# ZhiHuangHn/vtkCloudPoint

Measured on AMD Instinct MI355X. Metric: Mpoints/s DBSCAN+label @10M pts, higher is better.
Workload: dtype f64; 1 GPU; C4: 10000000-pt cloud (half uniform background, 200 Gaussian blobs), one monolithic DBImproved.dbscan, metric L1_2D, eps 0.1, minPts 10; mode=single, points_total=10000000, points_per_gpu=10000000, clusters=27380, resident_in_hbm=True

## Files before the change

### vtkcloudpoint_amd/csrc/gridbuild.hip

```cpp
#include <algorithm>
#include <mutex>
#include <unordered_map>

#include "grid_common.hpp"

using namespace vcpg;

namespace {

constexpr int PT = 1024;
constexpr int PCH_MIN = 8192;
constexpr int FT = 1024;
constexpr uint32_t MAXB = 8192;
constexpr uint32_t wcap(int) { return 4096u; }
constexpr uint32_t QUEUE_FROM = 32;

typedef float4 Rec;

template <int GD>
__device__ __forceinline__ Rec rec_make(const float* qf, uint32_t idx, uint32_t cell) {
  return GD == 2 ? make_float4(qf[0], qf[1], __uint_as_float(idx), __uint_as_float(cell))
                 : make_float4(qf[0], qf[1], qf[2], __uint_as_float(idx));
}
template <int GD>
// ... 27 lines not shown
  uint32_t nchunk;
};

inline int env_int(const char* name, int dflt, int lo, int hi) {
  const char* e = getenv(name);
  int v = e ? atoi(e) : dflt;
  return v < lo ? lo : v > hi ? hi : v;
}

inline PartGeom part_geom(int64_t n, uint32_t ncells) {
  static const int csh_max = env_int("VCP_CPB_LOG2", 14, 10, 14);
  static const int target = env_int("VCP_PART_CHUNKS", 256, 64, 8192);
  PartGeom p;
  int csh = csh_max;
  while (csh > 10 && ((uint64_t)ncells >> csh) * 4096ull < (uint64_t)n) csh--;
  p.csh = (uint32_t)csh;
  p.B = (uint32_t)((((uint64_t)ncells + 1) + ((1ull << p.csh) - 1)) >> p.csh);
  p.a = 0;
  while (((p.B + (1u << p.a) - 1u) >> p.a) > MAXB) p.a++;
  p.NS = (p.B + (1u << p.a) - 1u) >> p.a;
  int64_t chunk = (n + target - 1) / target;
  if (chunk < PCH_MIN) chunk = PCH_MIN;
  chunk = (chunk + PT - 1) / PT * PT;
  p.chunk = (uint32_t)chunk;
  p.nchunk = (uint32_t)((n + chunk - 1) / chunk);
  return p;
}

template <int GD, bool GROUPED>
__global__ __launch_bounds__(PT) void k_part_hist(const double* __restrict__ c, int64_t n, int stride, GridP g,
                                                 const int32_t* __restrict__ group, int glo, int ghi, uint32_t csh,
                                                 uint32_t B, uint32_t chunk, uint32_t nchunk,
                                                 uint32_t* __restrict__ counts, uint32_t* __restrict__ qcount,
                                                 uint32_t* __restrict__ ctcount) {
  extern __shared__ uint32_t h[];
  if (blockIdx.x == 0 && threadIdx.x == 0) {
    *qcount = 0u;
    ctcount[0] = 0u;
  }
  for (uint32_t k = threadIdx.x; k < B; k += PT) h[k] = 0;
  __syncthreads();
  const int64_t first = (int64_t)blockIdx.x * chunk;
  const int64_t last = min(first + (int64_t)chunk, n);
#pragma unroll 4
  for (int64_t i = first + threadIdx.x; i < last; i += PT) {
    if (GROUPED) {
      const int gg = group[i];
      if (gg < glo || gg >= ghi) continue;
    }
    float qf[3];
    atomicAdd(&h[point_cell<GD>(c, i, stride, g, qf) >> csh], 1u);
  }
  __syncthreads();
  for (uint32_t k = threadIdx.x; k < B; k += PT) counts[(size_t)k * nchunk + blockIdx.x] = h[k];
}

template <int GD, bool GROUPED>
__global__ __launch_bounds__(PT) void k_part_scatter(const double* __restrict__ c, int64_t n, int stride, GridP g,
                                                    const int32_t* __restrict__ group, int glo, int ghi, uint32_t csh,
                                                    uint32_t B, uint32_t chunk, uint32_t nchunk,
                                                    const uint32_t* __restrict__ base, Rec* __restrict__ rec,
                                                    uint32_t* __restrict__ pos) {
  extern __shared__ uint32_t h[];
  for (uint32_t k = threadIdx.x; k < B; k += PT) h[k] = base[(size_t)k * nchunk + blockIdx.x];
  __syncthreads();
  const int64_t first = (int64_t)blockIdx.x * chunk;
  const int64_t last = min(first + (int64_t)chunk, n);
#pragma unroll 4
  for (int64_t i = first + threadIdx.x; i < last; i += PT) {
    if (GROUPED) {
      const int gg = group[i];
      if (gg < glo || gg >= ghi) {
        if (pos) pos[i] = NONE;
        continue;
      }
    }
    float qf[3];
    const uint32_t cell = point_cell<GD>(c, i, stride, g, qf);
    rec[atomicAdd(&h[cell >> csh], 1u)] = rec_make<GD>(qf, (uint32_t)i, cell);
  }
}

__device__ __forceinline__ uint32_t padded(uint32_t i) { return i + (i >> 5); }

template <int GD, bool GROUPED, int NT = FT>
__device__ __forceinline__ void fine_flush(uint32_t s0, uint32_t m, const float* s32, const uint32_t* sidx,
                                           const uint32_t* __restrict__ ord, const uint8_t* __restrict__ in_classed,
                                           const int32_t* __restrict__ group, float* __restrict__ sorted32,
                                           uint32_t* __restrict__ sord, uint32_t* __restrict__ sidx_out,
                                           int32_t* __restrict__ sgroup, uint8_t* __restrict__ flags,
                                           uint32_t* __restrict__ pos) {
  if (GD == 2) {
    const float2* src = reinterpret_cast<const float2*>(s32);
    float2* dst = reinterpret_cast<float2*>(sorted32) + s0;
    for (uint32_t k = threadIdx.x; k < m; k += NT) dst[k] = src[k];
  } else {
    const float4* src = reinterpret_cast<const float4*>(s32);
    float4* dst = reinterpret_cast<float4*>(sorted32) + s0;
    for (uint32_t k = threadIdx.x; k < m; k += NT) dst[k] = src[k];
  }
  for (uint32_t k = threadIdx.x; k < m; k += NT) {
    const uint32_t i = sidx[k], p = s0 + k;
    sord[p] = ord ? ord[i] : i;
    if (sidx_out) sidx_out[p] = i;
    if (GROUPED) sgroup[p] = group[i];
    if (in_classed) flags[p] = in_classed[i] ? F_CLASSED : 0;
    if (pos) pos[i] = p;
  }
}

template <int GD>
__device__ __forceinline__ void stage_put(float* s32, uint32_t* sidx, uint32_t p, const Rec& r, uint32_t idx) {
  if (GD == 2) reinterpret_cast<float2*>(s32)[p] = make_float2(r.x, r.y);
  else reinterpret_cast<float4*>(s32)[p] = make_float4(r.x, r.y, r.z, 0.0f);
  sidx[p] = idx;
}

__device__ __forceinline__ void bucket_range(const uint32_t* __restrict__ bstart, uint32_t bstride, const uint32_t* __restrict__ total,
                                             uint32_t b, uint32_t B, uint32_t& s, uint32_t& e) {
  s = bstart[(size_t)b * bstride];
  e = (b + 1 < B) ? bstart[(size_t)(b + 1) * bstride] : *total;
}

template <int GD>
__global__ __launch_bounds__(FT) void k_part_split(const Rec* __restrict__ rec, Rec* __restrict__ rec2,
                                                  const uint32_t* __restrict__ base, const uint32_t* __restrict__ total,
                                                  uint32_t nchunk, uint32_t NS, uint32_t a, uint32_t csh, uint32_t B, GridP g,
                                                  uint32_t* __restrict__ bstart) {
  __shared__ uint32_t h[32];
  const uint32_t S = blockIdx.x;
  uint32_t s, e;
  bucket_range(base, nchunk, total, S, NS, s, e);
  const uint32_t subm = (1u << a) - 1u;
  if (threadIdx.x < 32) h[threadIdx.x] = 0u;
// ... 4 lines not shown
  }
  __syncthreads();
  if (threadIdx.x < 32) {
    const uint32_t v = h[threadIdx.x];
    uint32_t inc = v;
#pragma unroll
    for (int d = 1; d < 32; d <<= 1) {
      const uint32_t t = __shfl_up(inc, d, 64);
      if ((int)threadIdx.x >= d) inc += t;
    }
    const uint32_t first = s + inc - v;
    h[threadIdx.x] = first;
    const uint32_t bk = (S << a) + threadIdx.x;
    if (threadIdx.x <= subm && bk <= B) bstart[bk] = first;
  }
  __syncthreads();
  for (uint32_t j = s + threadIdx.x; j < e; j += FT) {
    const Rec r = rec[j];
    uint32_t i;
    rec2[atomicAdd(&h[(rec_cell<GD>(r, g, i) >> csh) & subm], 1u)] = r;
  }
}

constexpr int FS = 512;
constexpr uint32_t scap(int gd) { return gd == 2 ? 2048u : 1536u; }
constexpr uint32_t SPOP = 128;

template <int GD, bool GROUPED>
__global__ __launch_bounds__(FS) void k_part_fine_small(const Rec* __restrict__ rec, const uint32_t* __restrict__ bstart,
                                                       uint32_t bstride, const uint32_t* __restrict__ total, uint32_t B,
                                                       uint32_t csh, GridP g, const uint32_t* __restrict__ ord,
                                                       const uint8_t* __restrict__ in_classed, const int32_t* __restrict__ group,
                                                       uint4* __restrict__ ctwords, uint32_t* __restrict__ ctdense,
                                                       uint32_t* __restrict__ ctcount, uint8_t* __restrict__ bstate,
                                                       float* __restrict__ sorted32, uint32_t* __restrict__ sord,
                                                       uint32_t* __restrict__ sidx_out, int32_t* __restrict__ sgroup,
                                                       uint8_t* __restrict__ flags, uint32_t* __restrict__ pos) {
  constexpr uint32_t FPR = GD == 2 ? 2 : 4;
  constexpr uint32_t SCAP = scap(GD);
  constexpr int SRPT = SCAP / FS;
  __shared__ uint32_t ws[512 + 2];
  __shared__ uint32_t wlo[512], whi[512];
  __shared__ uint16_t wpi[512];
  __shared__ uint8_t sci[SCAP];
  __shared__ __attribute__((aligned(16))) uint16_t st32[SPOP][32];
  __shared__ __attribute__((aligned(16))) float s32[SCAP * FPR];
  __shared__ uint32_t sidx[SCAP];
  __shared__ uint32_t wsum[FS / 64];
  __shared__ uint32_t s_np, s_dbase;
  const uint32_t b = blockIdx.x;
  uint32_t s, e;
  bucket_range(bstart, bstride, total, b, B, s, e);
  const uint32_t m = e - s;
  if (b + 1 == B && threadIdx.x == 0) ctcount[1] = *total;
  if (m > SCAP) {
    if (threadIdx.x == 0) bstate[b] = 1;
    return;
  }
  const uint32_t CPB = 1u << csh, NW = CPB >> 5, c0 = b << csh;
  const int lane = threadIdx.x & 63, w = threadIdx.x >> 6;
  for (uint32_t k = threadIdx.x; k < NW + 1; k += FS) ws[k] = 0u;
  __syncthreads();
  Rec r[SRPT];
  uint32_t idx[SRPT], lw[SRPT], ci[SRPT], rnk[SRPT];
#pragma unroll
  for (int k = 0; k < SRPT; k++) {
    const uint32_t j = s + (uint32_t)k * FS + threadIdx.x;
    lw[k] = NONE;
    if (j < e) {
      r[k] = rec[j];
      const uint32_t c = rec_cell<GD>(r[k], g, idx[k]) - c0;
      lw[k] = c >> 5;
      ci[k] = c & 31u;
      rnk[k] = atomicAdd(&ws[lw[k]], 1u);
    }
  }
  __syncthreads();
  {
    const uint32_t v = threadIdx.x < NW ? ws[threadIdx.x] : 0u;
    uint32_t inc = v;
#pragma unroll
    for (int d = 1; d < 64; d <<= 1) {
      const uint32_t t = __shfl_up(inc, d, 64);
      if (lane >= d) inc += t;
    }
    if (lane == 63) wsum[w] = inc;
    __syncthreads();
    uint32_t pre = inc - v;
    for (int k = 0; k < w; k++) pre += wsum[k];
// ... 6 lines not shown
    if (lw[k] != NONE) sci[ws[lw[k]] - s + rnk[k]] = (uint8_t)ci[k];
  __syncthreads();
  bool popl = false;
  uint32_t lo = 0u, hi = 0u;
  if (threadIdx.x < NW) {
    const uint32_t a = ws[threadIdx.x] - s, k = ws[threadIdx.x + 1] - s - a;
    if (k > 64u) {
      popl = true;
    } else {
      for (uint32_t i = 0; i < k; i++) {
        const uint32_t bit = 1u << sci[a + i];
        if (lo & hi & bit) continue;
        if (lo & bit) hi ^= bit;
        lo ^= bit;
      }
      popl = (lo & hi) != 0u;
    }
  }
  {
    const unsigned long long dm = __ballot(popl);
    if (lane == 0) wsum[w] = (uint32_t)__popcll(dm);
    __syncthreads();
    uint32_t before = (uint32_t)__popcll(dm & ((1ull << lane) - 1ull)), tot = 0;
    for (int k = 0; k < FS / 64; k++) {
      if (k < w) before += wsum[k];
      tot += wsum[k];
    }
    if (threadIdx.x == 0) s_np = tot;
    if (threadIdx.x < NW) wpi[threadIdx.x] = popl ? (uint16_t)before : (uint16_t)0xFFFFu;
  }
  __syncthreads();
  const uint32_t np = s_np;
  if (np > SPOP) {
    if (threadIdx.x == 0) bstate[b] = 1;
    return;
  }
  if (threadIdx.x == 0) {
    bstate[b] = 0;
    s_dbase = np ? atomicAdd(&ctcount[0], np) : 0u;
  }
  for (uint32_t k = threadIdx.x; k < np * 16u; k += FS) reinterpret_cast<uint32_t*>(&st32[0][0])[k] = 0u;
  if (threadIdx.x < NW && !popl) {
    wlo[threadIdx.x] = lo;
    whi[threadIdx.x] = hi;
  }
  __syncthreads();
#pragma unroll
  for (int k = 0; k < SRPT; k++)
    if (lw[k] != NONE && wpi[lw[k]] != 0xFFFFu) {
      uint16_t* c = &st32[wpi[lw[k]]][ci[k]];
      atomicAdd(reinterpret_cast<uint32_t*>(reinterpret_cast<uintptr_t>(c) & ~(uintptr_t)3), ((uintptr_t)c & 2) ? 0x10000u : 1u);
    }
  __syncthreads();
  {
    const uint32_t hw = threadIdx.x >> 5, li = threadIdx.x & 31u;
    for (uint32_t wd = hw; wd < NW; wd += FS / 32) {
      const uint32_t pi = wpi[wd];
      if (pi == 0xFFFFu) continue;
      const uint32_t c = st32[pi][li];
      uint32_t inc = c;
#pragma unroll
      for (int d = 1; d < 32; d <<= 1) {
        const uint32_t t = __shfl_up(inc, d, 32);
        if ((int)li >= d) inc += t;
      }
      const uint32_t first = ws[wd] + inc - c;
      st32[pi][li] = (uint16_t)(first - s);
      ctdense[(size_t)(s_dbase + pi) * 32u + li] = first;
      const uint32_t cs = min(c, 3u);
      const unsigned long long blo = __ballot(cs & 1u), bhi = __ballot(cs >> 1);
      const int sh = (threadIdx.x & 32) ? 32 : 0;
      if (li == 0) {
        wlo[wd] = (uint32_t)(blo >> sh);
        whi[wd] = (uint32_t)(bhi >> sh);
      }
    }
  }
  __syncthreads();
#pragma unroll
  for (int k = 0; k < SRPT; k++) {
    if (lw[k] == NONE) continue;
    const uint32_t pi = wpi[lw[k]];
    uint32_t p;
    if (pi != 0xFFFFu) {
      uint16_t* c = &st32[pi][ci[k]];
      const bool up = ((uintptr_t)c & 2) != 0;
      const uint32_t old = atomicAdd(reinterpret_cast<uint32_t*>(reinterpret_cast<uintptr_t>(c) & ~(uintptr_t)3), up ? 0x10000u : 1u);
      p = up ? old >> 16 : old & 0xFFFFu;
    } else {
      const uint32_t l = wlo[lw[k]], h = whi[lw[k]], below = (1u << ci[k]) - 1u;
      const uint32_t a = ws[lw[k]] - s;
      p = a + (uint32_t)__popc(l & below) + 2u * (uint32_t)__popc(h & below);
      if ((h >> ci[k]) & 1u)
        for (uint32_t i = 0; i < rnk[k]; i++) p += sci[a + i] == (uint8_t)ci[k] ? 1u : 0u;
    }
    stage_put<GD>(s32, sidx, p, r[k], idx[k]);
  }
  if (threadIdx.x < NW) {
    const size_t W = (size_t)(c0 >> 5) + threadIdx.x;
    const uint32_t pi = wpi[threadIdx.x];
    if (W < vcp_ct_words(g.ncells))
      ctwords[W] = make_uint4(wlo[threadIdx.x], whi[threadIdx.x], ws[threadIdx.x], pi != 0xFFFFu ? s_dbase + pi : NONE);
  }
  __syncthreads();
  fine_flush<GD, GROUPED, FS>(s, m, s32, sidx, ord, in_classed, group, sorted32, sord, sidx_out, sgroup, flags, pos);
}

template <int GD, bool GROUPED>
__global__ __launch_bounds__(FT) void k_part_fine(const Rec* __restrict__ rec, uint32_t* __restrict__ rk,
                                                 const uint32_t* __restrict__ bstart, uint32_t bstride,
                                                 const uint32_t* __restrict__ total, uint32_t B, uint32_t csh, GridP g,
                                                 const uint32_t* __restrict__ ord, const uint8_t* __restrict__ in_classed,
                                                 const int32_t* __restrict__ group, uint4* __restrict__ ctwords,
                                                 uint32_t* __restrict__ ctdense, uint32_t* __restrict__ ctcount,
                                                 float* __restrict__ sorted32, uint32_t* __restrict__ sord,
                                                 uint32_t* __restrict__ sidx_out, int32_t* __restrict__ sgroup,
                                                 uint8_t* __restrict__ flags, uint32_t* __restrict__ pos,
                                                 uint2* __restrict__ queue, uint32_t* __restrict__ qcount,
                                                 const uint8_t* __restrict__ bstate) {
  extern __shared__ __attribute__((aligned(16))) unsigned char lds[];
  __shared__ uint32_t wsum[FT / 64];
  __shared__ uint32_t w_lo[512], w_hi[512], w_slot[512];
  __shared__ uint32_t s_dbase;
  const uint32_t b = blockIdx.x;
  if (bstate[b] == 0) return;
  constexpr uint32_t WCAP = wcap(GD);
  constexpr uint32_t FPR = GD == 2 ? 2 : 4;
  const uint32_t CPB = 1u << csh;
  uint32_t* cnt = reinterpret_cast<uint32_t*>(lds);
  float* s32 = reinterpret_cast<float*>(lds + (((size_t)padded(CPB) + 4) & ~3ull) * 4);
  uint32_t* sidx = reinterpret_cast<uint32_t*>(s32 + (size_t)WCAP * FPR);
  const uint32_t c0 = b << csh;
  uint32_t s, e;
  bucket_range(bstart, bstride, total, b, B, s, e);
  const uint32_t m = e - s;
  const bool big = m > WCAP;
  for (uint32_t k = threadIdx.x; k < padded(CPB); k += FT) cnt[k] = 0;
  __syncthreads();
  for (uint32_t j = s + threadIdx.x; j < e; j += FT) {
    uint32_t i;
    uint32_t* slot = &cnt[padded(rec_cell<GD>(rec[j], g, i) - c0)];
    if (big) rk[j] = atomicAdd(slot, 1u);
    else atomicAdd(slot, 1u);
  }
  __syncthreads();
  const uint32_t PER = CPB / FT;
  const uint32_t first = threadIdx.x * PER;
  uint32_t loc = 0;
  for (uint32_t k = 0; k < PER; k++) loc += cnt[padded(first + k)];
  const int lane = threadIdx.x & 63, w = threadIdx.x >> 6;
  uint32_t inc = loc;
#pragma unroll
  for (int d = 1; d < 64; d <<= 1) {
    const uint32_t t = __shfl_up(inc, d, 64);
    if (lane >= d) inc += t;
  }
  if (lane == 63) wsum[w] = inc;
  __syncthreads();
  uint32_t pre = s + inc - loc;
  for (int k = 0; k < w; k++) pre += wsum[k];
  const uint32_t NW = CPB >> 5;
  uint32_t plo = 0u, phi = 0u;
  const uint32_t wstart = pre;
  {
    const uint32_t bit0 = first & 31u;
    for (uint32_t k = 0; k < PER; k++) {
      const uint32_t v = cnt[padded(first + k)];
      cnt[padded(first + k)] = pre;
      pre += v;
      const uint32_t c = min(v, 3u);
      plo |= (c & 1u) << (bit0 + k);
      phi |= (c >> 1) << (bit0 + k);
    }
    for (uint32_t d = 1; d < 32u / PER; d <<= 1) {
      plo |= (uint32_t)__shfl_xor((int)plo, (int)d, 64);
      phi |= (uint32_t)__shfl_xor((int)phi, (int)d, 64);
    }
    if ((first & 31u) == 0u) {
      w_lo[first >> 5] = plo;
      w_hi[first >> 5] = phi;
      w_slot[first >> 5] = wstart;
    }
  }
  __syncthreads();
  {
    const bool popl = threadIdx.x < NW && (w_lo[threadIdx.x] & w_hi[threadIdx.x]) != 0u;
    const unsigned long long dm = __ballot(popl);
    if (lane == 0) wsum[w] = (uint32_t)__popcll(dm);
    __syncthreads();
    uint32_t before = (uint32_t)__popcll(dm & ((1ull << lane) - 1ull)), tot = 0;
    for (int k = 0; k < FT / 64; k++) {
      if (k < w) before += wsum[k];
      tot += wsum[k];
    }
    if (threadIdx.x == 0) s_dbase = tot ? atomicAdd(&ctcount[0], tot) : 0u;
    __syncthreads();
    if (threadIdx.x < NW) {
      const uint32_t slot = popl ? s_dbase + before : NONE;
      const uint32_t wpos = w_slot[threadIdx.x];
      w_slot[threadIdx.x] = slot;
      const size_t W = (size_t)(c0 >> 5) + threadIdx.x;
      if (W < vcp_ct_words(g.ncells))
        ctwords[W] = make_uint4(w_lo[threadIdx.x], w_hi[threadIdx.x], wpos, slot);
    }
    __syncthreads();
    const uint32_t hw = threadIdx.x >> 5, li = threadIdx.x & 31u;
    for (uint32_t j = hw; j < NW; j += FT / 32) {
      const uint32_t slot = w_slot[j];
      if (slot != NONE) ctdense[(size_t)slot * 32u + li] = cnt[padded(32u * j + li)];
    }
  }
  __syncthreads();
  if (!big) {
    for (uint32_t j = s + threadIdx.x; j < e; j += FT) {
      const Rec r = rec[j];
      uint32_t i;
      const uint32_t p = atomicAdd(&cnt[padded(rec_cell<GD>(r, g, i) - c0)], 1u) - s;
      stage_put<GD>(s32, sidx, p, r, i);
    }
    __syncthreads();
    fine_flush<GD, GROUPED>(s, m, s32, sidx, ord, in_classed, group, sorted32, sord, sidx_out, sgroup, flags, pos);
    return;
  }
  if (m > QUEUE_FROM * WCAP) {
    __shared__ uint32_t q0;
    const uint32_t nwin = (m + WCAP - 1) / WCAP;
    if (threadIdx.x == 0) q0 = atomicAdd(qcount, nwin);
    __syncthreads();
    for (uint32_t k = threadIdx.x; k < nwin; k += FT) queue[q0 + k] = make_uint2(b, k * WCAP);
    return;
  }
  for (uint32_t w0 = 0; w0 < m; w0 += WCAP) {
    for (uint32_t j = s + threadIdx.x; j < e; j += FT) {
      const Rec r = rec[j];
      uint32_t i;
      const uint32_t p = cnt[padded(rec_cell<GD>(r, g, i) - c0)] + rk[j] - s - w0;
      if (p < WCAP) stage_put<GD>(s32, sidx, p, r, i);
    }
    __syncthreads();
    fine_flush<GD, GROUPED>(s + w0, min(WCAP, m - w0), s32, sidx, ord, in_classed, group, sorted32, sord, sidx_out, sgroup,
                            flags, pos);
    __syncthreads();
  }
}

template <int GD, bool GROUPED>
__global__ __launch_bounds__(FT) void k_part_fine_windows(const Rec* __restrict__ rec, const uint32_t* __restrict__ rk,
                                                         const uint32_t* __restrict__ bstart, uint32_t bstride,
                                                         const uint32_t* __restrict__ total, uint32_t B, GridP g,
                                                         const uint32_t* __restrict__ ord, const uint8_t* __restrict__ in_classed,
                                                         const int32_t* __restrict__ group, CellTab ct,
                                                         float* __restrict__ sorted32,
                                                         uint32_t* __restrict__ sord, uint32_t* __restrict__ sidx_out,
                                                         int32_t* __restrict__ sgroup, uint8_t* __restrict__ flags,
                                                         uint32_t* __restrict__ pos, const uint2* __restrict__ queue,
                                                         const uint32_t* __restrict__ qcount) {
  extern __shared__ __attribute__((aligned(16))) unsigned char lds[];
  constexpr uint32_t WCAP = wcap(GD);
  constexpr uint32_t FPR = GD == 2 ? 2 : 4;
  float* s32 = reinterpret_cast<float*>(lds);
  uint32_t* sidx = reinterpret_cast<uint32_t*>(s32 + (size_t)WCAP * FPR);
  const uint32_t nq = *qcount;
  for (uint32_t qi = blockIdx.x; qi < nq; qi += gridDim.x) {
    const uint2 q = queue[qi];
    const uint32_t b = q.x, w0 = q.y;
    uint32_t s, e;
    bucket_range(bstart, bstride, total, b, B, s, e);
    const uint32_t m = e - s;
    for (uint32_t j = s + threadIdx.x; j < e; j += FT) {
      const Rec r = rec[j];
      uint32_t i;
      const uint32_t p = ct_start(ct, rec_cell<GD>(r, g, i)) + rk[j] - s - w0;
      if (p < WCAP) stage_put<GD>(s32, sidx, p, r, i);
    }
    __syncthreads();
    fine_flush<GD, GROUPED>(s + w0, min(WCAP, m - w0), s32, sidx, ord, in_classed, group, sorted32, sord, sidx_out, sgroup,
                            flags, pos);
    __syncthreads();
  }
}

constexpr int OT = 1024, OPT = 16;
constexpr int OWT = 512;

template <int OWSH>
__global__ __launch_bounds__(OT) void k_out_scatter(const uint32_t* __restrict__ sord, const uint32_t* __restrict__ labk,
                                                   int64_t n, uint32_t OB, uint32_t* __restrict__ gcur,
                                                   uint2* __restrict__ rec) {
  extern __shared__ uint32_t h[];
  for (uint32_t k = threadIdx.x; k < OB; k += OT) h[k] = 0;
  __syncthreads();
  const int64_t first = (int64_t)blockIdx.x * (OT * OPT);
  uint32_t o[OPT], w[OPT], r[OPT];
#pragma unroll
  for (int k = 0; k < OPT; k++) {
    const int64_t p = first + (int64_t)k * OT + threadIdx.x;
    o[k] = NONE;
    if (p < n) {
      o[k] = sord[p];
      w[k] = labk[p];
      r[k] = atomicAdd(&h[o[k] >> OWSH], 1u);
    }
  }
  __syncthreads();
  for (uint32_t k = threadIdx.x; k < OB; k += OT) {
    const uint32_t c = h[k];
    if (c) h[k] = atomicAdd(&gcur[k], c);
  }
  __syncthreads();
#pragma unroll
// ... 61 lines not shown
    }
  }
}

int allow_lds(vcp_ctx* ctx, const void* kernel, size_t bytes) {
  static std::mutex mu;
  static std::unordered_map<uint64_t, size_t> allowed;
  std::lock_guard<std::mutex> lk(mu);
  const uint64_t key = (uint64_t)reinterpret_cast<uintptr_t>(kernel) * 64u + (uint64_t)(ctx->device & 63);
  size_t& have = allowed.emplace(key, (size_t)64 * 1024).first->second;
  if (bytes > have) {
    VCP_HIP(ctx, hipFuncSetAttribute(kernel, hipFuncAttributeMaxDynamicSharedMemorySize, (int)bytes));
    have = bytes;
  }
  return VCP_OK;
}
template <class K>
int allow_lds(vcp_ctx* ctx, K kernel, size_t bytes) {
  return allow_lds(ctx, reinterpret_cast<const void*>(kernel), bytes);
}

template <int GD, bool GROUPED>
int build(vcp_ctx* ctx, const GridBuildArgs& a) {
  hipStream_t st = ctx->stream;
  const PartGeom pg = part_geom(a.n, a.g.ncells);
  const size_t nc = (size_t)pg.NS * pg.nchunk;
  VCP_TRY(vcp_ensure(ctx, ctx->b_hist, (nc + 8) * 4));
  VCP_TRY(vcp_ensure(ctx, ctx->b_rec, (size_t)a.n * sizeof(Rec)));
  uint32_t* counts = ctx->b_hist.as<uint32_t>();
  uint32_t* total = counts + nc;
  Rec* rec = ctx->b_rec.as<Rec>();
  const size_t lds_h = (size_t)pg.NS * 4;
  const uint32_t CPB = 1u << pg.csh;
  const size_t lds_f = ((((size_t)CPB + CPB / 32) + 4) & ~3ull) * 4 + (size_t)wcap(GD) * ((GD == 2 ? 8 : 16) + 4);
  VCP_TRY(allow_lds(ctx, k_part_fine<GD, GROUPED>, lds_f));
  VCP_TRY(vcp_ensure(ctx, ctx->b_fineq, ((size_t)a.n / wcap(GD) + pg.B + 8) * sizeof(uint2) + 64));
  uint32_t* qcount = ctx->b_fineq.as<uint32_t>();
  uint2* queue = reinterpret_cast<uint2*>(ctx->b_fineq.as<char>() + 64);
  vcp_phase(ctx, "part_hist");
  const uint32_t csh_a = pg.csh + pg.a;
  VCP_LAUNCH(ctx, (k_part_hist<GD, GROUPED>), dim3(pg.nchunk), dim3(PT), lds_h, st, a.d_coords, a.n, a.stride, a.g,
                  a.d_group, a.glo, a.ghi, csh_a, pg.NS, pg.chunk, pg.nchunk, counts, qcount, a.ctcount);
  VCP_TRY(vcp_exclusive_scan_u32(ctx, counts, counts, (int64_t)nc, total));
  vcp_phase(ctx, "part_scatter");
  VCP_LAUNCH(ctx, (k_part_scatter<GD, GROUPED>), dim3(pg.nchunk), dim3(PT), lds_h, st, a.d_coords, a.n, a.stride, a.g,
                  a.d_group, a.glo, a.ghi, csh_a, pg.NS, pg.chunk, pg.nchunk, counts, rec, a.pos);
  const uint32_t* bstart = counts;
  uint32_t bstride = pg.nchunk;
  if (pg.a > 0) {
    vcp_phase(ctx, "part_split");
    VCP_TRY(vcp_ensure(ctx, ctx->b_rec2, (size_t)a.n * sizeof(Rec)));
    VCP_TRY(vcp_ensure(ctx, ctx->b_bstart, ((size_t)pg.B + 2) * 4));
    VCP_LAUNCH(ctx, k_part_split<GD>, dim3(pg.NS), dim3(FT), 0, st, rec, ctx->b_rec2.as<Rec>(), counts, total, pg.nchunk,
                    pg.NS, pg.a, pg.csh, pg.B, a.g, ctx->b_bstart.as<uint32_t>());
    rec = ctx->b_rec2.as<Rec>();
    bstart = ctx->b_bstart.as<uint32_t>();
    bstride = 1;
  }
  vcp_phase(ctx, "part_fine");
  VCP_TRY(vcp_ensure(ctx, ctx->b_rank, (size_t)a.n * 4));
  VCP_TRY(vcp_ensure(ctx, ctx->b_bstate, (size_t)pg.B + 16));
  uint8_t* bstate = ctx->b_bstate.as<uint8_t>();
  VCP_LAUNCH(ctx, (k_part_fine_small<GD, GROUPED>), dim3(pg.B), dim3(FS), 0, st, rec, bstart, bstride, total, pg.B, pg.csh,
                  a.g, a.d_ord, a.d_in_classed, a.d_group, a.ctwords, a.ctdense, a.ctcount, bstate, a.sorted32, a.sord,
                  a.sidx, a.sgroup, a.flags, a.pos);
  VCP_LAUNCH(ctx, (k_part_fine<GD, GROUPED>), dim3(pg.B), dim3(FT), lds_f, st, rec, ctx->b_rank.as<uint32_t>(), bstart,
                  bstride, total, pg.B, pg.csh, a.g, a.d_ord, a.d_in_classed, a.d_group, a.ctwords, a.ctdense, a.ctcount,
                  a.sorted32, a.sord, a.sidx, a.sgroup, a.flags, a.pos, queue, qcount, bstate);
  {
    const size_t lds_w = (size_t)wcap(GD) * ((GD == 2 ? 8 : 16) + 4);
    VCP_TRY(allow_lds(ctx, k_part_fine_windows<GD, GROUPED>, lds_w));
    const unsigned gw = (unsigned)std::min<size_t>(768, (size_t)a.n / wcap(GD) + 1);
    const CellTab ct{a.ctwords, a.ctdense, a.ctcount + 1};
    VCP_LAUNCH(ctx, (k_part_fine_windows<GD, GROUPED>), dim3(gw), dim3(FT), lds_w, st, rec, ctx->b_rank.as<uint32_t>(),
                    bstart, bstride, total, pg.B, a.g, a.d_ord, a.d_in_classed, a.d_group, ct, a.sorted32,
                    a.sord, a.sidx, a.sgroup, a.flags, a.pos, queue, qcount);
  }
  return VCP_OK;
}

}

int vcp_grid_build_partition(vcp_ctx* ctx, const GridBuildArgs& a) {
  const bool grouped = a.d_group != nullptr;
  if (a.gd == 3) {
    if (grouped) return vcp_fail(ctx, VCP_ERR_ARG, "grouped calls are 2-D");
    return build<3, false>(ctx, a);
  }
  return grouped ? build<2, true>(ctx, a) : build<2, false>(ctx, a);
}

template <int OWSH>
static int output_partition(vcp_ctx* ctx, const GridOutputArgs& a) {
  hipStream_t st = ctx->stream;
  const uint32_t OB = (uint32_t)((a.n + (1 << OWSH) - 1) >> OWSH);
  const void* before = ctx->b_outcur.p;
  const size_t before_cap = ctx->b_outcur.cap;
  VCP_TRY(vcp_ensure(ctx, ctx->b_outcur, ((size_t)OB + 8) * 4));
  if (ctx->b_outcur.p != before || ctx->b_outcur.cap != before_cap)
    VCP_HIP(ctx, hipMemsetAsync(ctx->b_outcur.p, 0, ctx->b_outcur.cap, st));
  VCP_TRY(vcp_ensure(ctx, ctx->b_rec, (size_t)OB << (OWSH + 3)));
// ... 19 lines not shown
```

### vtkcloudpoint_amd/csrc/vcp_ctx.hpp

```cpp
#pragma once
#include <hip/hip_runtime.h>

#include <cstdarg>
#include <cstdint>
#include <cstdio>
#include <string>
#include <vector>

#include "vcp.h"

struct DevBuf {
  void* p = nullptr;
  size_t cap = 0;
  bool registered = false;
  template <class T>
  T* as() const { return reinterpret_cast<T*>(p); }
};

struct Phase {
  const char* name;
  hipEvent_t ev;
};

struct vcp_ctx {
  int device = 0;
  hipStream_t own_stream = nullptr;
  hipStream_t stream = nullptr;
  std::string err;
  hipDeviceProp_t prop;
  void* pinned = nullptr;
  size_t pinned_bytes = 0;
  void* stage = nullptr;
  size_t stage_bytes = 0;
  uint32_t scan_gen = 0;
  std::vector<DevBuf*> bufs;
  DevBuf b_cellof, b_rank, b_sidx, b_flags, b_parent, b_minord, b_seedflag,
      b_rootcl, b_clseed, b_scan_tmp, b_misc, b_in0, b_in1, b_in2, b_in3, b_out0, b_out1, b_out2,
      b_out3, b_icp_part, b_aux0, b_aux1, b_aux2, b_aux3, b_aux4, b_aux5, b_pos, b_labk, b_sgroup, b_wl, b_hist, b_rec, b_nn_misc, b_nn_cells, b_nn_cid, b_nn_rec, b_nn_cur, b_nbr, b_nboff, b_sorted32, b_self, b_outcur, b_fineq, b_rec2, b_bstart, b_ctw, b_ctd, b_bstate;
  DevBuf b_kd_in, b_kd_out, b_kd_outk, b_kd_part, b_kd_key, b_kd_val, b_kd_rec, b_kd_start, b_kd_heavy, b_kd_tmp;
  DevBuf b_sh_hull, b_sh_out, b_sh_flag;
  DevBuf b_mu_cent, b_mu_truth, b_mu_misc, b_mu_cell;
  DevBuf b_rg_in, b_rg_truth, b_rg_cell, b_rg_work;
  DevBuf b_et_in, b_et_out, b_et_kd, b_et_misc, b_et_cell, b_et_work, b_et_edge, b_et_tmp;
  DevBuf b_gd_in, b_gd_out, b_gd_misc, b_gd_cell, b_gd_work;
  DevBuf b_icpt;
  struct BlocksState* blocks = nullptr;
  struct SlabState* slab = nullptr;
  bool timing = false;
  std::vector<Phase> phases;
  std::vector<hipEvent_t> ev_pool;
  size_t ev_used = 0;
  std::vector<std::pair<const char*, float>> last_timing;
};

int vcp_fail(vcp_ctx* ctx, int code, const char* fmt, ...);
void* vcp_stage(vcp_ctx* ctx, size_t bytes);

#define VCP_HIP(ctx, call)                                                                    \
  do {                                                                                        \
    hipError_t e__ = (call);                                                                  \
    if (e__ != hipSuccess)                                                                    \
      return vcp_fail((ctx), VCP_ERR_HIP, "%s:%d %s -> %s", __FILE__, __LINE__, #call,        \
                      hipGetErrorString(e__));                                                \
  } while (0)

#define VCP_TRY(expr)        \
  do {                       \
    int rc__ = (expr);       \
    if (rc__ != VCP_OK) return rc__; \
  } while (0)

// ... 42 lines not shown
```

Measured before the change: 7016 Mpoints/s.

## Make fine partition kernel persistent over a compacted list of dense buckets

Buckets that overflow the small-bucket kernel are now pushed onto a compact device list through an atomic head, replacing the per-bucket state byte. The large fine kernel is launched with one block per CU and loops over that list through a work-stealing counter, prefetching the next bucket's records into registers while the current one finishes. It also keeps up to eight records per thread in registers instead of re-reading them and writing ranks, uses DPP wave scans and lighter LDS barriers, and changes LDS padding to keep 16-byte aligned vector access. This removes launching and early-exiting thousands of empty blocks, at the cost of more register pressure and serialising dense buckets onto fewer blocks.

```diff
diff --git a/vtkcloudpoint_amd/csrc/gridbuild.hip b/vtkcloudpoint_amd/csrc/gridbuild.hip
--- a/vtkcloudpoint_amd/csrc/gridbuild.hip
+++ b/vtkcloudpoint_amd/csrc/gridbuild.hip
@@ -83,11 +83,13 @@
                                                  const int32_t* __restrict__ group, int glo, int ghi, uint32_t csh,
                                                  uint32_t B, uint32_t chunk, uint32_t nchunk,
                                                  uint32_t* __restrict__ counts, uint32_t* __restrict__ qcount,
-                                                 uint32_t* __restrict__ ctcount) {
+                                                 uint32_t* __restrict__ ctcount, uint32_t* __restrict__ dhead) {
   extern __shared__ uint32_t h[];
   if (blockIdx.x == 0 && threadIdx.x == 0) {
     *qcount = 0u;
     ctcount[0] = 0u;
+    dhead[0] = 0u;
+    dhead[1] = 0u;
   }
   for (uint32_t k = threadIdx.x; k < B; k += PT) h[k] = 0;
   __syncthreads();
@@ -132,7 +134,7 @@
   }
 }
 
-__device__ __forceinline__ uint32_t padded(uint32_t i) { return i + (i >> 5); }
+__device__ __forceinline__ uint32_t padded(uint32_t i) { return i + ((i >> 6) << 2); }
 
 template <int GD, bool GROUPED, int NT = FT>
 __device__ __forceinline__ void fine_flush(uint32_t s0, uint32_t m, const float* s32, const uint32_t* sidx,
@@ -140,17 +142,17 @@
                                            const int32_t* __restrict__ group, float* __restrict__ sorted32,
                                            uint32_t* __restrict__ sord, uint32_t* __restrict__ sidx_out,
                                            int32_t* __restrict__ sgroup, uint8_t* __restrict__ flags,
-                                           uint32_t* __restrict__ pos) {
+                                           uint32_t* __restrict__ pos, uint32_t tid) {
   if (GD == 2) {
     const float2* src = reinterpret_cast<const float2*>(s32);
     float2* dst = reinterpret_cast<float2*>(sorted32) + s0;
-    for (uint32_t k = threadIdx.x; k < m; k += NT) dst[k] = src[k];
+    for (uint32_t k = tid; k < m; k += NT) dst[k] = src[k];
   } else {
     const float4* src = reinterpret_cast<const float4*>(s32);
     float4* dst = reinterpret_cast<float4*>(sorted32) + s0;
-    for (uint32_t k = threadIdx.x; k < m; k += NT) dst[k] = src[k];
-  }
-  for (uint32_t k = threadIdx.x; k < m; k += NT) {
+    for (uint32_t k = tid; k < m; k += NT) dst[k] = src[k];
+  }
+  for (uint32_t k = tid; k < m; k += NT) {
     const uint32_t i = sidx[k], p = s0 + k;
     sord[p] = ord ? ord[i] : i;
     if (sidx_out) sidx_out[p] = i;
@@ -221,7 +223,8 @@
                                                        uint32_t csh, GridP g, const uint32_t* __restrict__ ord,
                                                        const uint8_t* __restrict__ in_classed, const int32_t* __restrict__ group,
                                                        uint4* __restrict__ ctwords, uint32_t* __restrict__ ctdense,
-                                                       uint32_t* __restrict__ ctcount, uint8_t* __restrict__ bstate,
+                                                       uint32_t* __restrict__ ctcount, uint32_t* __restrict__ dhead,
+                                                       uint4* __restrict__ dlist,
                                                        float* __restrict__ sorted32, uint32_t* __restrict__ sord,
                                                        uint32_t* __restrict__ sidx_out, int32_t* __restrict__ sgroup,
                                                        uint8_t* __restrict__ flags, uint32_t* __restrict__ pos) {
@@ -243,7 +246,7 @@
   const uint32_t m = e - s;
   if (b + 1 == B && threadIdx.x == 0) ctcount[1] = *total;
   if (m > SCAP) {
-    if (threadIdx.x == 0) bstate[b] = 1;
+    if (threadIdx.x == 0) dlist[atomicAdd(&dhead[1], 1u)] = make_uint4(b, s, e, 0u);
     return;
   }
   const uint32_t CPB = 1u << csh, NW = CPB >> 5, c0 = b << csh;
@@ -316,13 +319,10 @@
   __syncthreads();
   const uint32_t np = s_np;
   if (np > SPOP) {
-    if (threadIdx.x == 0) bstate[b] = 1;
+    if (threadIdx.x == 0) dlist[atomicAdd(&dhead[1], 1u)] = make_uint4(b, s, e, 0u);
     return;
   }
-  if (threadIdx.x == 0) {
-    bstate[b] = 0;
-    s_dbase = np ? atomicAdd(&ctcount[0], np) : 0u;
-  }
+  if (threadIdx.x == 0) s_dbase = np ? atomicAdd(&ctcount[0], np) : 0u;
   for (uint32_t k = threadIdx.x; k < np * 16u; k += FS) reinterpret_cast<uint32_t*>(&st32[0][0])[k] = 0u;
   if (threadIdx.x < NW && !popl) {
     wlo[threadIdx.x] = lo;
@@ -387,144 +387,245 @@
       ctwords[W] = make_uint4(wlo[threadIdx.x], whi[threadIdx.x], ws[threadIdx.x], pi != 0xFFFFu ? s_dbase + pi : NONE);
   }
   __syncthreads();
-  fine_flush<GD, GROUPED, FS>(s, m, s32, sidx, ord, in_classed, group, sorted32, sord, sidx_out, sgroup, flags, pos);
+  fine_flush<GD, GROUPED, FS>(s, m, s32, sidx, ord, in_classed, group, sorted32, sord, sidx_out, sgroup, flags, pos,
+                              threadIdx.x);
+}
+
+constexpr int FRPT = 8;
+#ifndef VCP_FINE_PERSIST
+#define VCP_FINE_PERSIST 1
+#endif
+
+template <int GD>
+__device__ __forceinline__ uint32_t rec_idx(const Rec& r) {
+  return __float_as_uint(GD == 2 ? r.z : r.w);
+}
+
+template <int K0, int K1>
+__device__ __forceinline__ void fine_load(const Rec* __restrict__ rec, uint32_t s, uint32_t e, uint32_t tid, Rec* r) {
+#pragma unroll
+  for (int k = K0; k < K1; k++) r[k - K0] = rec[min(s + (uint32_t)k * FT + tid, e - 1u)];
+}
+
+__device__ __forceinline__ void lds_barrier() { asm volatile("s_waitcnt lgkmcnt(0)\n\ts_barrier" ::: "memory"); }
+
+__device__ __forceinline__ uint32_t wave_scan(uint32_t x) {
+  int v = (int)x;
+  v += __builtin_amdgcn_update_dpp(0, v, 0x111, 0xf, 0xf, false);
+  v += __builtin_amdgcn_update_dpp(0, v, 0x112, 0xf, 0xf, false);
+  v += __builtin_amdgcn_update_dpp(0, v, 0x114, 0xf, 0xf, false);
+  v += __builtin_amdgcn_update_dpp(0, v, 0x118, 0xf, 0xf, false);
+  v += __builtin_amdgcn_update_dpp(0, v, 0x142, 0xa, 0xf, false);
+  v += __builtin_amdgcn_update_dpp(0, v, 0x143, 0xc, 0xf, false);
+  return (uint32_t)v;
+}
+
+__device__ __forceinline__ uint4 dense_entry(const uint4* __restrict__ dlist, uint32_t t, uint32_t nd) {
+  uint32_t b = NONE, s = 0u, e = 0u;
+  if (t < nd) {
+    const uint4 v = dlist[t];
+    b = v.x, s = v.y, e = v.z;
+  }
+  return make_uint4(b, s, e, 0u);
 }
 
 template <int GD, bool GROUPED>
-__global__ __launch_bounds__(FT) void k_part_fine(const Rec* __restrict__ rec, uint32_t* __restrict__ rk,
-                                                 const uint32_t* __restrict__ bstart, uint32_t bstride,
-                                                 const uint32_t* __restrict__ total, uint32_t B, uint32_t csh, GridP g,
-                                                 const uint32_t* __restrict__ ord, const uint8_t* __restrict__ in_classed,
+__global__ __launch_bounds__(FT) void k_part_fine(const Rec* __restrict__ rec, uint32_t* __restrict__ rk, uint32_t csh,
+                                                 GridP g, const uint32_t* __restrict__ ord,
+                                                 const uint8_t* __restrict__ in_classed,
                                                  const int32_t* __restrict__ group, uint4* __restrict__ ctwords,
                                                  uint32_t* __restrict__ ctdense, uint32_t* __restrict__ ctcount,
                                                  float* __restrict__ sorted32, uint32_t* __restrict__ sord,
                                                  uint32_t* __restrict__ sidx_out, int32_t* __restrict__ sgroup,
                                                  uint8_t* __restrict__ flags, uint32_t* __restrict__ pos,
                                                  uint2* __restrict__ queue, uint32_t* __restrict__ qcount,
-                                                 const uint8_t* __restrict__ bstate) {
+                                                 uint32_t* __restrict__ dhead, const uint4* __restrict__ dlist) {
   extern __shared__ __attribute__((aligned(16))) unsigned char lds[];
   __shared__ uint32_t wsum[FT / 64];
   __shared__ uint32_t w_lo[512], w_hi[512], w_slot[512];
-  __shared__ uint32_t s_dbase;
-  const uint32_t b = blockIdx.x;
-  if (bstate[b] == 0) return;
+  __shared__ uint32_t s_dbase, s_q0;
+  __shared__ uint4 s_ent[2];
   constexpr uint32_t WCAP = wcap(GD);
   constexpr uint32_t FPR = GD == 2 ? 2 : 4;
-  const uint32_t CPB = 1u << csh;
+  constexpr uint32_t CAPR = (uint32_t)FT * FRPT;
+  constexpr int FPRE = GD == 2 ? 4 : 2;
+  const uint32_t CPB = 1u << csh, NW = CPB >> 5, PER = CPB / FT;
   uint32_t* cnt = reinterpret_cast<uint32_t*>(lds);
   float* s32 = reinterpret_cast<float*>(lds + (((size_t)padded(CPB) + 4) & ~3ull) * 4);
   uint32_t* sidx = reinterpret_cast<uint32_t*>(s32 + (size_t)WCAP * FPR);
-  const uint32_t c0 = b << csh;
-  uint32_t s, e;
-  bucket_range(bstart, bstride, total, b, B, s, e);
-  const uint32_t m = e - s;
-  const bool big = m > WCAP;
+  const uint32_t nd = dhead[1];
+  uint32_t tq = NONE;
+  uint4 entn = make_uint4(NONE, 0u, 0u, 0u);
+  if (threadIdx.x == 0) s_ent[0] = dense_entry(dlist, atomicAdd(&dhead[0], 1u), nd);
   for (uint32_t k = threadIdx.x; k < padded(CPB); k += FT) cnt[k] = 0;
   __syncthreads();
-  for (uint32_t j = s + threadIdx.x; j < e; j += FT) {
-    uint32_t i;
-    uint32_t* slot = &cnt[padded(rec_cell<GD>(rec[j], g, i) - c0)];
-    if (big) rk[j] = atomicAdd(slot, 1u);
-    else atomicAdd(slot, 1u);
-  }
-  __syncthreads();
-  const uint32_t PER = CPB / FT;
-  const uint32_t first = threadIdx.x * PER;
-  uint32_t loc = 0;
-  for (uint32_t k = 0; k < PER; k++) loc += cnt[padded(first + k)];
-  const int lane = threadIdx.x & 63, w = threadIdx.x >> 6;
-  uint32_t inc = loc;
-#pragma unroll
-  for (int d = 1; d < 64; d <<= 1) {
-    const uint32_t t = __shfl_up(inc, d, 64);
-    if (lane >= d) inc += t;
-  }
-  if (lane == 63) wsum[w] = inc;
-  __syncthreads();
-  uint32_t pre = s + inc - loc;
-  for (int k = 0; k < w; k++) pre += wsum[k];
-  const uint32_t NW = CPB >> 5;
-  uint32_t plo = 0u, phi = 0u;
-  const uint32_t wstart = pre;
-  {
-    const uint32_t bit0 = first & 31u;
-    for (uint32_t k = 0; k < PER; k++) {
-      const uint32_t v = cnt[padded(first + k)];
-      cnt[padded(first + k)] = pre;
-      pre += v;
-      const uint32_t c = min(v, 3u);
-      plo |= (c & 1u) << (bit0 + k);
-      phi |= (c >> 1) << (bit0 + k);
-    }
-    for (uint32_t d = 1; d < 32u / PER; d <<= 1) {
-      plo |= (uint32_t)__shfl_xor((int)plo, (int)d, 64);
-      phi |= (uint32_t)__shfl_xor((int)phi, (int)d, 64);
-    }
-    if ((first & 31u) == 0u) {
-      w_lo[first >> 5] = plo;
-      w_hi[first >> 5] = phi;
-      w_slot[first >> 5] = wstart;
-    }
-  }
-  __syncthreads();
-  {
-    const bool popl = threadIdx.x < NW && (w_lo[threadIdx.x] & w_hi[threadIdx.x]) != 0u;
+  uint4 cur = s_ent[0];
+  if (cur.x == NONE) return;
+  Rec R[FRPT], N[FPRE];
+  fine_load<0, FPRE>(rec, cur.y, cur.z, threadIdx.x, R);
+  if (VCP_FINE_PERSIST && threadIdx.x == 0) entn = dense_entry(dlist, atomicAdd(&dhead[0], 1u), nd);
+  for (;;) {
+    uint32_t tid = threadIdx.x;
+    asm volatile("" : "+v"(tid));
+    const int lane = tid & 63, w = tid >> 6;
+    const uint32_t b = cur.x, s = cur.y, e = cur.z, m = e - s, c0 = b << csh;
+    const bool inreg = m <= CAPR;
+    const bool queued = m > QUEUE_FROM * WCAP;
+    if (tid == 0) s_ent[1] = entn;
+    if (FPRE < FRPT && inreg && m > (uint32_t)FPRE * FT) fine_load<FPRE, FRPT>(rec, s, e, tid, R + FPRE);
+    uint32_t rnk[FRPT];
+    auto cell_at = [&](int k) {
+      uint32_t i;
+      return rec_cell<GD>(R[k], g, i) - c0;
+    };
+#pragma unroll
+    for (int k = 0; k < FRPT; k++) {
+      rnk[k] = NONE;
+      if (inreg && s + (uint32_t)k * FT + tid < e) rnk[k] = atomicAdd(&cnt[padded(cell_at(k))], 1u);
+    }
+    if (!inreg)
+      for (uint32_t j = s + tid; j < e; j += FT) {
+        uint32_t i;
+        rk[j] = atomicAdd(&cnt[padded(rec_cell<GD>(rec[j], g, i) - c0)], 1u);
+      }
+    if (inreg) lds_barrier();
+    else __syncthreads();
+    const uint4 nxt = s_ent[1];
+    tq = NONE;
+    if (tid == 0 && nxt.x != NONE) tq = atomicAdd(&dhead[0], 1u);
+    if (nxt.x != NONE) fine_load<0, FPRE>(rec, nxt.y, nxt.z, tid, N);
+    const uint32_t first = tid * PER;
+    uint32_t loc = 0;
+    if (PER >= 4u) {
+      const uint4* c4 = reinterpret_cast<const uint4*>(cnt + padded(first));
+#pragma unroll
+      for (uint32_t q = 0; q < 4; q++) {
+        if (q * 4u >= PER) break;
+        const uint4 x = c4[q];
+        loc += x.x + x.y + x.z + x.w;
+      }
+    } else {
+      for (uint32_t k = 0; k < PER; k++) loc += cnt[padded(first + k)];
+    }
+    const uint32_t inc = wave_scan(loc);
+    if (lane == 63) wsum[w] = inc;
+    lds_barrier();
+    uint32_t pre = s + inc - loc;
+#pragma unroll
+    for (int k = 0; k < FT / 64; k++) pre += k < w ? wsum[k] : 0u;
+    uint32_t plo = 0u, phi = 0u;
+    const uint32_t wstart = pre;
+    {
+      const uint32_t bit0 = first & 31u;
+      auto cell = [&](uint32_t v, uint32_t k) {
+        const uint32_t at = pre, c = min(v, 3u);
+        pre += v;
+        plo |= (c & 1u) << (bit0 + k);
+        phi |= (c >> 1) << (bit0 + k);
+        return at;
+      };
+      if (PER >= 4u) {
+        uint4* c4 = reinterpret_cast<uint4*>(cnt + padded(first));
+#pragma unroll
+        for (uint32_t q = 0; q < 4; q++) {
+          if (q * 4u >= PER) break;
+          const uint4 x = c4[q];
+          uint4 st;
+          st.x = cell(x.x, 4u * q);
+          st.y = cell(x.y, 4u * q + 1u);
+          st.z = cell(x.z, 4u * q + 2u);
+          st.w = cell(x.w, 4u * q + 3u);
+          c4[q] = st;
+        }
+      } else {
+        for (uint32_t k = 0; k < PER; k++) cnt[padded(first + k)] = cell(cnt[padded(first + k)], k);
+      }
+      if (PER < 32u) {
+        plo |= (uint32_t)__builtin_amdgcn_update_dpp(0, (int)plo, 0xB1, 0xf, 0xf, false);
+        phi |= (uint32_t)__builtin_amdgcn_update_dpp(0, (int)phi, 0xB1, 0xf, 0xf, false);
+      }
+      for (uint32_t d = 2; d < 32u / PER; d <<= 1) {
+        plo |= (uint32_t)__shfl_xor((int)plo, (int)d, 64);
+        phi |= (uint32_t)__shfl_xor((int)phi, (int)d, 64);
+      }
+      if ((first & 31u) == 0u) {
+        w_lo[first >> 5] = plo;
+        w_hi[first >> 5] = phi;
+        w_slot[first >> 5] = wstart;
+      }
+    }
+    lds_barrier();
+    auto stage = [&](uint32_t w0) {
+      if (inreg) {
+#pragma unroll
+        for (int k = 0; k < FRPT; k++) {
+          if (rnk[k] == NONE) continue;
+          const uint32_t p = cnt[padded(cell_at(k))] + rnk[k] - s - w0;
+          if (p < WCAP) stage_put<GD>(s32, sidx, p, R[k], rec_idx<GD>(R[k]));
+        }
+      } else {
+        for (uint32_t j = s + tid; j < e; j += FT) {
+          const Rec r = rec[j];
+          uint32_t i;
+          const uint32_t p = cnt[padded(rec_cell<GD>(r, g, i) - c0)] + rk[j] - s - w0;
+          if (p < WCAP) stage_put<GD>(s32, sidx, p, r, i);
+        }
+      }
+    };
+    const bool popl = tid < NW && (w_lo[tid] & w_hi[tid]) != 0u;
     const unsigned long long dm = __ballot(popl);
     if (lane == 0) wsum[w] = (uint32_t)__popcll(dm);
-    __syncthreads();
+    lds_barrier();
     uint32_t before = (uint32_t)__popcll(dm & ((1ull << lane) - 1ull)), tot = 0;
     for (int k = 0; k < FT / 64; k++) {
       if (k < w) before += wsum[k];
       tot += wsum[k];
     }
-    if (threadIdx.x == 0) s_dbase = tot ? atomicAdd(&ctcount[0], tot) : 0u;
-    __syncthreads();
-    if (threadIdx.x < NW) {
+    uint32_t dbase = 0u;
+    if (tid == 0 && tot) dbase = atomicAdd(&ctcount[0], tot);
+    const uint32_t nwin = (m + WCAP - 1) / WCAP;
+    if (!queued) stage(0u);
+    if (tid == 0) {
+      s_dbase = dbase;
+      if (queued) s_q0 = atomicAdd(qcount, nwin);
+      entn = dense_entry(dlist, tq, nd);
+    }
+    lds_barrier();
+    if (tid < NW) {
       const uint32_t slot = popl ? s_dbase + before : NONE;
-      const uint32_t wpos = w_slot[threadIdx.x];
-      w_slot[threadIdx.x] = slot;
-      const size_t W = (size_t)(c0 >> 5) + threadIdx.x;
-      if (W < vcp_ct_words(g.ncells))
-        ctwords[W] = make_uint4(w_lo[threadIdx.x], w_hi[threadIdx.x], wpos, slot);
-    }
-    __syncthreads();
-    const uint32_t hw = threadIdx.x >> 5, li = threadIdx.x & 31u;
-    for (uint32_t j = hw; j < NW; j += FT / 32) {
-      const uint32_t slot = w_slot[j];
-      if (slot != NONE) ctdense[(size_t)slot * 32u + li] = cnt[padded(32u * j + li)];
-    }
-  }
-  __syncthreads();
-  if (!big) {
-    for (uint32_t j = s + threadIdx.x; j < e; j += FT) {
-      const Rec r = rec[j];
-      uint32_t i;
-      const uint32_t p = atomicAdd(&cnt[padded(rec_cell<GD>(r, g, i) - c0)], 1u) - s;
-      stage_put<GD>(s32, sidx, p, r, i);
-    }
-    __syncthreads();
-    fine_flush<GD, GROUPED>(s, m, s32, sidx, ord, in_classed, group, sorted32, sord, sidx_out, sgroup, flags, pos);
-    return;
-  }
-  if (m > QUEUE_FROM * WCAP) {
-    __shared__ uint32_t q0;
-    const uint32_t nwin = (m + WCAP - 1) / WCAP;
-    if (threadIdx.x == 0) q0 = atomicAdd(qcount, nwin);
-    __syncthreads();
-    for (uint32_t k = threadIdx.x; k < nwin; k += FT) queue[q0 + k] = make_uint2(b, k * WCAP);
-    return;
-  }
-  for (uint32_t w0 = 0; w0 < m; w0 += WCAP) {
-    for (uint32_t j = s + threadIdx.x; j < e; j += FT) {
-      const Rec r = rec[j];
-      uint32_t i;
-      const uint32_t p = cnt[padded(rec_cell<GD>(r, g, i) - c0)] + rk[j] - s - w0;
-      if (p < WCAP) stage_put<GD>(s32, sidx, p, r, i);
-    }
-    __syncthreads();
-    fine_flush<GD, GROUPED>(s + w0, min(WCAP, m - w0), s32, sidx, ord, in_classed, group, sorted32, sord, sidx_out, sgroup,
-                            flags, pos);
-    __syncthreads();
+      const uint32_t wpos = w_slot[tid];
+      w_slot[tid] = slot;
+      const size_t W = (size_t)(c0 >> 5) + tid;
+      if (W < vcp_ct_words(g.ncells)) ctwords[W] = make_uint4(w_lo[tid], w_hi[tid], wpos, slot);
+    }
+    lds_barrier();
+    {
+      const uint32_t hw = tid >> 5, li = tid & 31u;
+      for (uint32_t j = hw; j < NW; j += FT / 32) {
+        const uint32_t slot = w_slot[j];
+        if (slot != NONE) ctdense[(size_t)slot * 32u + li] = cnt[padded(32u * j + li)];
+      }
+    }
+    if (queued) {
+      for (uint32_t k = tid; k < nwin; k += FT) queue[s_q0 + k] = make_uint2(b, k * WCAP);
+    } else {
+      for (uint32_t w0 = 0;;) {
+        fine_flush<GD, GROUPED>(s + w0, min(WCAP, m - w0), s32, sidx, ord, in_classed, group, sorted32, sord, sidx_out,
+                                sgroup, flags, pos, tid);
+        w0 += WCAP;
+        if (w0 >= m) break;
+        lds_barrier();
+        stage(w0);
+        lds_barrier();
+      }
+    }
+    if (nxt.x == NONE) break;
+    lds_barrier();
+    for (uint32_t k = tid; k < (padded(CPB) + 3u) / 4u; k += FT) reinterpret_cast<uint4*>(cnt)[k] = make_uint4(0u, 0u, 0u, 0u);
+    lds_barrier();
+    cur = nxt;
+#pragma unroll
+    for (int k = 0; k < FPRE; k++) R[k] = N[k];
   }
 }
 
@@ -559,7 +660,7 @@
     }
     __syncthreads();
     fine_flush<GD, GROUPED>(s + w0, min(WCAP, m - w0), s32, sidx, ord, in_classed, group, sorted32, sord, sidx_out, sgroup,
-                            flags, pos);
+                            flags, pos, threadIdx.x);
     __syncthreads();
   }
 }
@@ -687,15 +788,18 @@
   Rec* rec = ctx->b_rec.as<Rec>();
   const size_t lds_h = (size_t)pg.NS * 4;
   const uint32_t CPB = 1u << pg.csh;
-  const size_t lds_f = ((((size_t)CPB + CPB / 32) + 4) & ~3ull) * 4 + (size_t)wcap(GD) * ((GD == 2 ? 8 : 16) + 4);
+  const size_t lds_f = ((((size_t)CPB + CPB / 16) + 4) & ~3ull) * 4 + (size_t)wcap(GD) * ((GD == 2 ? 8 : 16) + 4);
   VCP_TRY(allow_lds(ctx, k_part_fine<GD, GROUPED>, lds_f));
   VCP_TRY(vcp_ensure(ctx, ctx->b_fineq, ((size_t)a.n / wcap(GD) + pg.B + 8) * sizeof(uint2) + 64));
   uint32_t* qcount = ctx->b_fineq.as<uint32_t>();
   uint2* queue = reinterpret_cast<uint2*>(ctx->b_fineq.as<char>() + 64);
+  VCP_TRY(vcp_ensure(ctx, ctx->b_dense, 16 + (size_t)pg.B * sizeof(uint4)));
+  uint32_t* dhead = ctx->b_dense.as<uint32_t>();
+  uint4* dlist = reinterpret_cast<uint4*>(dhead + 4);
   vcp_phase(ctx, "part_hist");
   const uint32_t csh_a = pg.csh + pg.a;
   VCP_LAUNCH(ctx, (k_part_hist<GD, GROUPED>), dim3(pg.nchunk), dim3(PT), lds_h, st, a.d_coords, a.n, a.stride, a.g,
-                  a.d_group, a.glo, a.ghi, csh_a, pg.NS, pg.chunk, pg.nchunk, counts, qcount, a.ctcount);
+                  a.d_group, a.glo, a.ghi, csh_a, pg.NS, pg.chunk, pg.nchunk, counts, qcount, a.ctcount, dhead);
   VCP_TRY(vcp_exclusive_scan_u32(ctx, counts, counts, (int64_t)nc, total));
   vcp_phase(ctx, "part_scatter");
   VCP_LAUNCH(ctx, (k_part_scatter<GD, GROUPED>), dim3(pg.nchunk), dim3(PT), lds_h, st, a.d_coords, a.n, a.stride, a.g,
@@ -714,14 +818,13 @@
   }
   vcp_phase(ctx, "part_fine");
   VCP_TRY(vcp_ensure(ctx, ctx->b_rank, (size_t)a.n * 4));
-  VCP_TRY(vcp_ensure(ctx, ctx->b_bstate, (size_t)pg.B + 16));
-  uint8_t* bstate = ctx->b_bstate.as<uint8_t>();
   VCP_LAUNCH(ctx, (k_part_fine_small<GD, GROUPED>), dim3(pg.B), dim3(FS), 0, st, rec, bstart, bstride, total, pg.B, pg.csh,
-                  a.g, a.d_ord, a.d_in_classed, a.d_group, a.ctwords, a.ctdense, a.ctcount, bstate, a.sorted32, a.sord,
+                  a.g, a.d_ord, a.d_in_classed, a.d_group, a.ctwords, a.ctdense, a.ctcount, dhead, dlist, a.sorted32, a.sord,
                   a.sidx, a.sgroup, a.flags, a.pos);
-  VCP_LAUNCH(ctx, (k_part_fine<GD, GROUPED>), dim3(pg.B), dim3(FT), lds_f, st, rec, ctx->b_rank.as<uint32_t>(), bstart,
-                  bstride, total, pg.B, pg.csh, a.g, a.d_ord, a.d_in_classed, a.d_group, a.ctwords, a.ctdense, a.ctcount,
-                  a.sorted32, a.sord, a.sidx, a.sgroup, a.flags, a.pos, queue, qcount, bstate);
+  const unsigned gf = VCP_FINE_PERSIST ? std::min<unsigned>(pg.B, (unsigned)std::max(ctx->prop.multiProcessorCount, 1)) : pg.B;
+  VCP_LAUNCH(ctx, (k_part_fine<GD, GROUPED>), dim3(gf), dim3(FT), lds_f, st, rec, ctx->b_rank.as<uint32_t>(), pg.csh, a.g,
+                  a.d_ord, a.d_in_classed, a.d_group, a.ctwords, a.ctdense, a.ctcount, a.sorted32, a.sord, a.sidx, a.sgroup,
+                  a.flags, a.pos, queue, qcount, dhead, dlist);
   {
     const size_t lds_w = (size_t)wcap(GD) * ((GD == 2 ? 8 : 16) + 4);
     VCP_TRY(allow_lds(ctx, k_part_fine_windows<GD, GROUPED>, lds_w));
diff --git a/vtkcloudpoint_amd/csrc/vcp_ctx.hpp b/vtkcloudpoint_amd/csrc/vcp_ctx.hpp
--- a/vtkcloudpoint_amd/csrc/vcp_ctx.hpp
+++ b/vtkcloudpoint_amd/csrc/vcp_ctx.hpp
@@ -36,7 +36,7 @@
   std::vector<DevBuf*> bufs;
   DevBuf b_cellof, b_rank, b_sidx, b_flags, b_parent, b_minord, b_seedflag,
       b_rootcl, b_clseed, b_scan_tmp, b_misc, b_in0, b_in1, b_in2, b_in3, b_out0, b_out1, b_out2,
-      b_out3, b_icp_part, b_aux0, b_aux1, b_aux2, b_aux3, b_aux4, b_aux5, b_pos, b_labk, b_sgroup, b_wl, b_hist, b_rec, b_nn_misc, b_nn_cells, b_nn_cid, b_nn_rec, b_nn_cur, b_nbr, b_nboff, b_sorted32, b_self, b_outcur, b_fineq, b_rec2, b_bstart, b_ctw, b_ctd, b_bstate;
+      b_out3, b_icp_part, b_aux0, b_aux1, b_aux2, b_aux3, b_aux4, b_aux5, b_pos, b_labk, b_sgroup, b_wl, b_hist, b_rec, b_nn_misc, b_nn_cells, b_nn_cid, b_nn_rec, b_nn_cur, b_nbr, b_nboff, b_sorted32, b_self, b_outcur, b_fineq, b_rec2, b_bstart, b_ctw, b_ctd, b_dense;
   DevBuf b_kd_in, b_kd_out, b_kd_outk, b_kd_part, b_kd_key, b_kd_val, b_kd_rec, b_kd_start, b_kd_heavy, b_kd_tmp;
   DevBuf b_sh_hull, b_sh_out, b_sh_flag;
   DevBuf b_mu_cent, b_mu_truth, b_mu_misc, b_mu_cell;
```

Measured after the change: 7101 Mpoints/s (median of 6 runs). +1.2%, better.
